# thevasudevgupta/gsoc-wav2vec2

Measured on AMD Instinct MI355X. Metric: audio-seconds/s (wav2vec2-base forward, 246000-sample pad), higher is better.
Workload: dtype f32

## Files before the change

gsoc-wav2vec2_amd/csrc/common.h:

```cpp
#pragma once

#include <hip/hip_runtime.h>
#include <stdint.h>
#include <stdio.h>

#include <atomic>
#include <initializer_list>
#include <type_traits>

#include <string>

#include "../../include/w2v2.h"

namespace w2v2 {

void set_error(const char* fmt, ...);

#define W2V2_HIP_CHECK(expr)                                                            \
    do {                                                                                \
        hipError_t _e = (expr);                                                         \
        if (_e != hipSuccess) {                                                         \
            ::w2v2::set_error("%s failed: %s (%s:%d)", #expr, hipGetErrorString(_e),    \
                              __FILE__, __LINE__);                                      \
            return W2V2_EHIP;                                                           \
// ... 95 lines not shown
    int outer_family;
    ProfScope(Profiler* p_, int family, double flops, double bytes, hipStream_t s_)
        : p(p_), tok((p_ && tl_prof_depth == 0) ? profiler_begin(p_, family, flops, bytes, s_) : -1), s(s_), outer_family(tl_launch_family) {
        if (tl_prof_depth++ == 0) tl_launch_family = family;
    }
    ~ProfScope() {
        if (--tl_prof_depth == 0) tl_launch_family = outer_family;
        if (tok >= 0) profiler_end(p, tok, s);
    }
};

extern thread_local Profiler* tl_step_prof;
struct StepProfScope {
    Profiler* outer;
    explicit StepProfScope(Profiler* p) : outer(tl_step_prof) { tl_step_prof = p; }
    ~StepProfScope() { tl_step_prof = outer; }
};

int launch_gemm(Profiler* prof, const float* A, int64_t lda, int64_t strideA, const float* B,
                int64_t ldb, float* C, int64_t ldc, int64_t strideC, const float* bias,
                const float* residual, int M, int N, int K, int nbatch, int act, hipStream_t s);

void gemm_f32_force_ring(int route);
bool gemm_f32_ring_ok(int tile, const float* A, int64_t lda, int64_t strideA, const float* B, int64_t ldb, int64_t strideB,
                      int M, int N, int K);
int launch_gemm_f32_ring(int tile, bool persist, const float* A, int64_t lda, int64_t strideA, const float* B, int64_t ldb,
                         int64_t strideB, float* C, int64_t ldc, int64_t strideC, const float* bias, const float* residual, int M,
                         int N, int K, int nbatch, int act, hipStream_t s);
int launch_gemm_f32_ring_split(bool persist, int64_t main_tiles, const float* A, int64_t lda, const float* B, int64_t ldb, float* C,
                               int64_t ldc, const float* bias, const float* residual, int M, int N, int K, int act, hipStream_t s);

int launch_gemm_bf16(Profiler* prof, const float* A, int64_t lda, int64_t strideA, const float* B, int64_t ldb,
                     int64_t strideB, float* C, int64_t ldc, int64_t strideC, const float* bias,
                     const float* residual, int M, int N, int K, int nbatch, int act, hipStream_t s);
bool gemm_split_supported(const float* A, int64_t lda, int64_t strideA, int M, int N, int K);
int launch_split_weight(const float* w, uint16_t* planes, int K, int N, hipStream_t s);
int launch_gemm_split(Profiler* prof, const float* A, int64_t lda, int64_t strideA, const uint16_t* planes, float* C, int64_t ldc,
                      int64_t strideC, const float* bias, const float* residual, int M, int N, int K, int nbatch, int act,
                      hipStream_t s);

bool gemm_split_sw_ok(const uint16_t* A16, int64_t planeA, int64_t lda, int64_t strideA, int M, int N, int K);
int launch_split_weight_sw(const float* w, uint16_t* img, int K, int N, int fmt, void* scratch, hipStream_t s);
int launch_split_planes(const float* x, uint16_t* planes, int64_t plane, int64_t n, int fmt, int* range_flag, hipStream_t s);
int launch_gemm_split_sw(Profiler* prof, int fmt, const uint16_t* A16, int64_t planeA, int64_t lda, int64_t strideA, const uint16_t* Bimg,
                         const float* out_scale, float* C, uint16_t* C16, int64_t planeC, int64_t ldc, int64_t strideC, const float* bias,
                         const float* residual, int M, int N, int K, int nbatch, int act, int* range_flag, hipStream_t s);

int launch_check_select_forms(unsigned long long* mismatches_dev , hipStream_t s);

struct GemmShadows {
    const uint16_t* A16 = nullptr;
    const uint16_t* B16 = nullptr;
    uint16_t* C16 = nullptr;
    int64_t ldb16 = 0;
    bool transA = false;
    int zmod = 0;
    int64_t strideB16 = 0, strideC2 = 0, strideBias = 0;
    int64_t strideB2 = 0;
    bool overlapA = false;
    int kseg = 0;
    int64_t segA = 0, segB = 0;
    float* colsum = nullptr;
    int64_t strideCS = 0;
    const uint16_t* B16p = nullptr;
    int64_t validK = 0;
    int kextra = 0;
    bool b_zero_row = false;
    int force_kernel = 0;
};
bool gemm_bf16_sw_ok(int M, int N, int K, int64_t lda, int64_t ldb16, int64_t strideA);
int launch_gemm_bf16_sw(const uint16_t* A16, int64_t lda, int64_t strideA, const uint16_t* B16, int64_t ldb16, float* C, uint16_t* C16,
// ... 207 lines not shown
    q = __builtin_fmaf(ax, q, 0x1.4515fap-1f);
    q = __builtin_fmaf(ax, q, 0x1.078e5p-3f);
    q = __builtin_fmaf(ax, q, ax);
    const float large = 1.0f - expf(-q);
    return copysignf(ax < 1.0f ? small : large, x);
}
__device__ __forceinline__ float tanh_select(float x) {
    const float ax = fabsf(x), t = x * x;
    float p = __builtin_fmaf(t, -0x1.758e7ap-8f, 0x1.521192p-6f);
    p = __builtin_fmaf(t, p, -0x1.b8389cp-5f);
    p = __builtin_fmaf(t, p, 0x1.110704p-3f);
    p = __builtin_fmaf(t, p, -0x1.555532p-2f);
    const float small = __builtin_fmaf(t, ax * p, ax);
    const float large = __builtin_fmaf(-2.0f, __builtin_amdgcn_rcpf(expf(ax * 2.0f) + 1.0f), 1.0f);
    return copysignf(ax < 0.625f ? small : large, x);
}
__device__ __forceinline__ float gelu_tanh_select(float x) {
    const float c = 0.79788456080286535588f;
    return 0.5f * x * (1.0f + tanh_select(c * (x + 0.044715f * x * x * x)));
}
__device__ __forceinline__ float gelu_erf_select(float x) {
    return 0.5f * x * (1.0f + erf_select(x * 0.70710678118654752440f));
}
__device__ __forceinline__ float gelu_tanh(float x) {
    const float c = 0.79788456080286535588f;
    return 0.5f * x * (1.0f + tanhf(c * (x + 0.044715f * x * x * x)));
}
__device__ __forceinline__ float gelu_erf_fast(float x) {
    const float z = fabsf(x) * 0.70710678118654752440f;
    const float t = __builtin_amdgcn_rcpf(fmaf(0.3275911f, z, 1.0f));
    float p = fmaf(1.061405429f, t, -1.453152027f);
    p = fmaf(p, t, 1.421413741f);
    p = fmaf(p, t, -0.284496736f);
    p = fmaf(p, t, 0.254829592f);
    const float e = __builtin_amdgcn_exp2f(-z * z * 1.44269504088896340736f);
    const float erf_abs = fmaf(-p * t, e, 1.0f);
    return 0.5f * x + 0.5f * fabsf(x) * erf_abs;
}

using f32x2_t = __attribute__((ext_vector_type(2))) float;
__device__ __forceinline__ f32x2_t gelu_erf_fast2(f32x2_t x) {
    const f32x2_t ax = {fabsf(x[0]), fabsf(x[1])};
    const f32x2_t z = ax * f32x2_t{0.70710678118654752440f, 0.70710678118654752440f};
    const f32x2_t d = __builtin_elementwise_fma(f32x2_t{0.3275911f, 0.3275911f}, z, f32x2_t{1.0f, 1.0f});
    const f32x2_t t = {__builtin_amdgcn_rcpf(d[0]), __builtin_amdgcn_rcpf(d[1])};
    f32x2_t q = __builtin_elementwise_fma(f32x2_t{1.061405429f, 1.061405429f}, t, f32x2_t{-1.453152027f, -1.453152027f});
// ... 105 lines not shown
```

gsoc-wav2vec2_amd/csrc/gemm_epilogue.h:

```cpp
#pragma once

#include "common.h"
#include "train.h"

namespace w2v2 {

#ifdef __HIPCC__
using f32x16_t = __attribute__((ext_vector_type(16))) float;

template <int MT, int NTL, bool FAST_GELU>
__device__ __forceinline__ void gemm_epilogue(const f32x16_t (&acc)[MT][NTL], float* __restrict__ C, uint16_t* __restrict__ C16,
                                              const float* __restrict__ R, const float* __restrict__ bias, int ldc,
                                              int rows_left, int cols_left, int act, int li, int lh, int64_t c16_plane = 0, int c16_fmt = 0,
                                              int* range_flag = nullptr) {
    bool ovf = false;
    const bool interior = rows_left >= MT * 32 && cols_left >= NTL * 32;
#pragma unroll
    for (int nt = 0; nt < NTL; ++nt) {
        const int cl = nt * 32 + li;
        const bool col_ok = cl < cols_left;
        const float bv = (bias && col_ok) ? bias[cl] : 0.0f;
#pragma unroll
        for (int mt = 0; mt < MT; ++mt) {
            f32x16_t v = acc[mt][nt];
#pragma unroll
            for (int r = 0; r < 16; ++r) v[r] += bv;
            if (act == 1) {
#pragma unroll
                for (int r = 0; r < 16; r += 2) {
                    if (FAST_GELU) {
                        const f32x2_t g = gelu_erf_fast2(f32x2_t{v[r], v[r + 1]});
                        v[r] = g[0];
                        v[r + 1] = g[1];
                    } else {
                        v[r] = gelu_erf(v[r]);
                        v[r + 1] = gelu_erf(v[r + 1]);
                    }
                }
            } else if (act == 2) {
#pragma unroll
                for (int r = 0; r < 16; ++r) v[r] = gelu_tanh(v[r]);
            }
            const int off0 = (mt * 32 + 4 * lh) * ldc + cl;
            if (interior) {
                if (R) {
#pragma unroll
                    for (int r = 0; r < 16; ++r) v[r] += R[off0 + ((r & 3) + 8 * (r >> 2)) * ldc];
                }
                if (C) {
#pragma unroll
                    for (int r = 0; r < 16; ++r) C[off0 + ((r & 3) + 8 * (r >> 2)) * ldc] = v[r];
                }
                if (C16) {
#pragma unroll
                    for (int r = 0; r < 16; ++r) {
                        uint16_t* const d = C16 + off0 + ((r & 3) + 8 * (r >> 2)) * ldc;
                        if (c16_plane && c16_fmt == PF_F16X2) split2h_one(v[r], F16X2_ACT_SCALE, d[0], d[c16_plane], ovf);
                        else if (c16_plane) split3_one(v[r], d[0], d[c16_plane], d[2 * c16_plane]);
                        else d[0] = (uint16_t)pack_bf16_rne(v[r], 0.0f);
                    }
                }
            } else if (col_ok) {
#pragma unroll
                for (int r = 0; r < 16; ++r) {
                    const int rl = mt * 32 + (r & 3) + 8 * (r >> 2) + 4 * lh;
                    if (rl < rows_left) {
                        const int off = off0 + ((r & 3) + 8 * (r >> 2)) * ldc;
                        float o = v[r];
                        if (R) o += R[off];
                        if (C) C[off] = o;
// ... 17 lines not shown
```

gsoc-wav2vec2_amd/csrc/gemm_f32.hip:

```cpp
#include <stdlib.h>


#include "common.h"
#include "gemm_epilogue.h"

namespace w2v2 {

using f32x16 = __attribute__((ext_vector_type(16))) float;
using f32x4 = __attribute__((ext_vector_type(4))) float;

namespace {

constexpr int BK = 32;
constexpr int LDA_S = BK + 4;

struct GemmArgs {
    const float* A;
    const float* B;
    float* C;
    const float* bias;
    const float* residual;
    int64_t lda, ldb, ldc, strideA, strideB, strideC;
    int M, N, K, act;
    int tiles_m, tiles_n;
// ... 324 lines not shown
    const int64_t n4 = (int64_t)M * N / 4;
    for (int64_t i = (int64_t)blockIdx.x * 256 + threadIdx.x; i < n4; i += (int64_t)gridDim.x * 256) {
        const int64_t e = i * 4, row = e / N;
        const int col = (int)(e % N);
        float4 acc = reinterpret_cast<const float4*>(slabs)[i];
        for (int z = 1; z < S; ++z) {
            const float4 v = reinterpret_cast<const float4*>(slabs + (int64_t)z * M * N)[i];
            acc.x += v.x; acc.y += v.y; acc.z += v.z; acc.w += v.w;
        }
        if (bias) { acc.x += bias[col]; acc.y += bias[col + 1]; acc.z += bias[col + 2]; acc.w += bias[col + 3]; }
        acc.x = apply_act(acc.x, act); acc.y = apply_act(acc.y, act); acc.z = apply_act(acc.z, act); acc.w = apply_act(acc.w, act);
        if (residual) {
            const float4 r = *reinterpret_cast<const float4*>(residual + row * ldc + col);
            acc.x += r.x; acc.y += r.y; acc.z += r.z; acc.w += r.w;
        }
        *reinterpret_cast<float4*>(C + row * ldc + col) = acc;
    }
}

thread_local int tl_precision = 0;
thread_local int tl_ring = -1;

constexpr int RING_DEFAULT = 2;
int ring_route() { return tl_ring >= 0 ? tl_ring : tune_int("W2V2_GEMM_RING", RING_DEFAULT); }

}

void gemm_set_precision(int mode) { tl_precision = mode; }
void gemm_f32_force_ring(int route) { tl_ring = route; }
int gemm_get_precision() { return tl_precision; }

int launch_gemm(Profiler* prof, const float* A, int64_t lda, int64_t strideA, const float* B,
                int64_t ldb, float* C, int64_t ldc, int64_t strideC, const float* bias,
                const float* residual, int M, int N, int K, int nbatch, int act, hipStream_t s) {
    return launch_gemm_ex(prof, A, lda, strideA, B, ldb, 0, C, ldc, strideC, bias, residual, M, N, K, nbatch, act, s);
}

int launch_gemm_ex(Profiler* prof, const float* A, int64_t lda, int64_t strideA, const float* B,
                   int64_t ldb, int64_t strideB, float* C, int64_t ldc, int64_t strideC, const float* bias,
                   const float* residual, int M, int N, int K, int nbatch, int act, hipStream_t s) {
    if (tl_precision == 1)
        return launch_gemm_bf16(prof, A, lda, strideA, B, ldb, strideB, C, ldc, strideC, bias, residual, M, N, K, nbatch, act, s);
    W2V2_REQUIRE(A && B && C, "gemm: null operand");
    W2V2_REQUIRE(M > 0 && N > 0 && K > 0 && nbatch > 0, "gemm: bad sizes M=%d N=%d K=%d batch=%d", M, N, K, nbatch);
    W2V2_REQUIRE(lda >= 1 && ldb >= N && ldc >= N && ldc < (1 << 23), "gemm: bad leading dimensions");
    W2V2_REQUIRE(act >= 0 && act <= 2, "gemm: bad activation %d", act);
    GemmArgs g;
    g.A = A; g.B = B; g.C = C; g.bias = bias; g.residual = residual;
    g.lda = lda; g.ldb = ldb; g.ldc = ldc; g.strideA = strideA; g.strideB = strideB; g.strideC = strideC;
    g.M = M; g.N = N; g.K = K; g.act = act;
    const bool fast = (K % BK == 0) && (N % 4 == 0) && (lda % 4 == 0) && (ldb % 4 == 0) &&
                      (strideA % 4 == 0) && (strideB % 4 == 0) && ((reinterpret_cast<uintptr_t>(A) & 15) == 0) &&
                      ((reinterpret_cast<uintptr_t>(B) & 15) == 0);
    ProfScope ps(prof, FAM_GEMM, 2.0 * M * (double)N * K * nbatch,
                 4.0 * nbatch * ((double)M * K + (double)M * N) + 4.0 * (double)K * N, s);
    int cfg = forced_cfg();
    const bool by_shape = cfg < 0;
    if (cfg < 0 && fast && nbatch == 1 && strideB == 0 && K >= 1024 && (ldc % 4) == 0 &&
        ((reinterpret_cast<uintptr_t>(C) | reinterpret_cast<uintptr_t>(residual) | reinterpret_cast<uintptr_t>(bias)) & 15) == 0) {
        const int64_t tiles64 = (int64_t)((M + 63) / 64) * ((N + 63) / 64);
        int S = 1;
        for (int cand = 8; cand >= 2; cand >>= 1)
            if (K % (cand * BK) == 0 && K / cand >= 256 && tiles64 * cand <= 512) { S = cand; break; }
        if (S > 1 && tiles64 <= 256) {
            const size_t need = (size_t)S * M * N;
            float* ws = nullptr;
            void* raw = nullptr;
            if (int e = stream_scratch(SCRATCH_SPLITK, s, need * sizeof(float), &raw)) return e;
            ws = reinterpret_cast<float*>(raw);
            GemmArgs h = g;
            h.C = ws; h.bias = nullptr; h.residual = nullptr; h.act = 0;
            h.K = K / S; h.strideA = K / S; h.strideB = (int64_t)(K / S) * ldb; h.ldc = N; h.strideC = (int64_t)M * N;
            if (int e = launch_dma<2, 2, 2, 32, 64, 64>(h, S, s)) return e;
            const int64_t n4 = (int64_t)M * N / 4;
            int64_t blocks = (n4 + 255) / 256;
            blocks = blocks > 2048 ? 2048 : blocks;
            W2V2_LAUNCH(splitk_reduce_kernel, dim3((unsigned)blocks), dim3(256), 0, s, ws, C, bias, residual, M, N, ldc, S, act);
            W2V2_HIP_CHECK(hipGetLastError());
// ... 87 lines not shown
```

gsoc-wav2vec2_amd/csrc/gemm_f32_sw.hip:

```cpp
#include "common.h"
#include "gemm_epilogue.h"
#include "gemm_sw_common.h"

namespace w2v2 {

namespace {

struct GemmRingArgs {
    const float* A;
    const float* B;
    float* C;
    const float* bias;
    const float* residual;
    int64_t lda, ldb, ldc, strideA, strideB, strideC;
    int M, N, K, act;
    int tiles_m, tiles_n, nbatch;
    int gm;
    int total;
    int first;
};

template <int WM, int WN, int BKT, int BM, int BN, int NS>
struct RingCfg {
    static constexpr int STAGE = (BM * BKT + BKT * BN) * 4;
    static constexpr int LDS = NS * STAGE;
    static constexpr int NW = WM * WN;
    static constexpr int NPA = BM * BKT / 256, NPB = BKT * BN / 256;
    static constexpr int PPA = NPA / NW, PPB = NPB / NW;
    static constexpr int P = PPA + PPB;
    static_assert(NPA % NW == 0 && NPB % NW == 0, "every wave issues the same number of pieces (counted waits)");
    static_assert((NS - 2) * P <= 63, "vmcnt field");
};

template <int WM, int WN, int BKT, int BM, int BN, int NS, bool QUAD = false>
__global__ __launch_bounds__(WM* WN * 64) __attribute__((amdgpu_waves_per_eu(4))) void gemm_f32_ring_kernel(GemmRingArgs g) {
    using R_ = RingCfg<WM, WN, BKT, BM, BN, NS>;
    constexpr int NW = R_::NW, PPA = R_::PPA, PPB = R_::PPB, P = R_::P, STAGE = R_::STAGE;
    constexpr int RPP = 256 / BKT;
    constexpr int SPR = BKT / 4;
    constexpr int SW = BKT == 32 ? 1 : 2;
    constexpr int WTM = BM / WM, WTN = BN / WN, MT = WTM / 32, NTL = WTN / 32;
    extern __shared__ __attribute__((aligned(16))) float smem[];
    const int tid = threadIdx.x, lane = tid & 63, wave = __builtin_amdgcn_readfirstlane(tid >> 6);
    const int wm = wave / WN, wn = wave % WN, li = lane & 31, lh = lane >> 5;
    const unsigned lds0 = (unsigned)(uintptr_t)(__attribute__((address_space(3))) float*)smem;

    const int nwg = g.tiles_m * g.tiles_n, total = g.total, G = gridDim.x;
    const int ntl = (total - (int)blockIdx.x + G - 1) / G;
    const int nk = g.K / BKT, nsteps = ntl * nk;
    auto tile_of = [&](int i, int& z, int& m0, int& n0) {
        const int v = (int)blockIdx.x + i * G;
        const int q = total >> 3, r = total & 7, xcd = v & 7, idx = v >> 3;
        int t = (xcd < r ? xcd * (q + 1) : r * (q + 1) + (xcd - r) * q) + idx;
        int sub = 0;
        if constexpr (QUAD) {
            sub = t & 3;
            t = g.first + (t >> 2);
// ... 89 lines not shown
#pragma unroll
                for (int mt = 0; mt < MT; ++mt)
#pragma unroll
                    for (int nt = 0; nt < NTL; ++nt)
                        acc[mt][nt] = __builtin_amdgcn_mfma_f32_32x32x2f32(a[mt][e], b[nt][e], acc[mt][nt], 0, 0, 0);
        }
    };
    auto ring_barrier = [&](bool counted) {
        if (counted) sw_wait_vm<(NS - 2) * P>();
        else sw_wait_vm<0>();
        __builtin_amdgcn_s_barrier();
        asm volatile("" ::: "memory");
        __builtin_amdgcn_sched_barrier(0);
    };

    set_issue_tile(0);
    for (int p = 0; p < NS - 1 && p < nsteps; ++p) issue_step();
    ring_barrier(nsteps >= NS - 1);
    __builtin_amdgcn_s_setprio(1);

    int s = 0, cst = 0;
    for (int ci = 0; ci < ntl; ++ci) {
        zero();
        for (int kt = 0; kt < nk; ++kt, ++s) {
            const bool more = s + NS - 1 < nsteps;
            if (more) issue_step();
            __builtin_amdgcn_sched_barrier(0);
            compute(cst);
            __builtin_amdgcn_sched_barrier(0);
            ring_barrier(more);
            cst = cst + 1 == NS ? 0 : cst + 1;
        }
        int z, m0, n0;
        tile_of(ci, z, m0, n0);
        const int64_t tile_off = (int64_t)z * g.strideC + (int64_t)(m0 + wm * WTM) * g.ldc + (n0 + wn * WTN);
        int act = g.act, ldc = (int)g.ldc, eli = li, elh = lh;
        const float* res = g.residual;
        const float* bias = g.bias;
        asm volatile("" : "+s"(act), "+s"(res), "+s"(bias), "+s"(ldc), "+v"(eli), "+v"(elh));
        __builtin_amdgcn_s_setprio(0);
        gemm_epilogue<MT, NTL, false>(acc, g.C + tile_off, nullptr, res ? res + tile_off : nullptr, bias ? bias + (n0 + wn * WTN) : nullptr,
                                     ldc, g.M - (m0 + wm * WTM), g.N - (n0 + wn * WTN), act, eli, elh);
        __builtin_amdgcn_s_setprio(1);
    }
    __builtin_amdgcn_s_setprio(0);
}

template <int WM, int WN, int BKT, int BM, int BN, int NS, bool QUAD = false>
int launch_ring(GemmRingArgs& g, bool persist, hipStream_t s, int64_t first = -1, int gm = 0) {
    using R_ = RingCfg<WM, WN, BKT, BM, BN, NS>;
    static_assert(2 * R_::LDS <= 160 * 1024, "two blocks per CU");
    constexpr int TM = QUAD ? 2 * BM : BM, TN = QUAD ? 2 * BN : BN;
    g.tiles_m = (g.M + TM - 1) / TM;
    g.tiles_n = (g.N + TN - 1) / TN;
    int64_t total = (int64_t)g.tiles_m * g.tiles_n * g.nbatch;
    W2V2_REQUIRE(first < 0 || (first > 0 && first < total && g.nbatch == 1 && g.M % TM == 0 && g.N % TN == 0), "gemm ring: bad split");
    W2V2_REQUIRE(!QUAD || first > 0, "gemm ring: quarter tiles need a split");
    g.first = QUAD ? (int)first : 0;
    if (first > 0) total = QUAD ? 4 * (total - first) : first;
    W2V2_REQUIRE(total < (1ll << 31), "gemm ring: %lld tiles", (long long)total);
    g.total = (int)total;
    constexpr int PER_CU = WM * WN == 8 ? 2 : 160 * 1024 / R_::LDS > 4 ? 4 : 160 * 1024 / R_::LDS;
    int grid = (int)total;
    if (persist) {
        int dev = 0, cus = 0;
        W2V2_HIP_CHECK(hipGetDevice(&dev));
        W2V2_HIP_CHECK(hipDeviceGetAttribute(&cus, hipDeviceAttributeMultiprocessorCount, dev));
        const int resident = (PER_CU * cus) & ~7;
        if (resident >= 8 && total > resident) grid = resident;
    }
    g.gm = first > 0 ? gm : g.nbatch == 1 ? tile_group_rows(g.tiles_m, g.tiles_n, (int64_t)BM * g.K * 4, BM == 256 ? 96 : 32 * PER_CU) : 0;
    static std::atomic<bool> attr_set{false};
    if (!attr_set) {
        W2V2_HIP_CHECK(hipFuncSetAttribute(reinterpret_cast<const void*>(gemm_f32_ring_kernel<WM, WN, BKT, BM, BN, NS, QUAD>),
                                           hipFuncAttributeMaxDynamicSharedMemorySize, R_::LDS));
        attr_set = true;
    }
    W2V2_LAUNCH((gemm_f32_ring_kernel<WM, WN, BKT, BM, BN, NS, QUAD>), dim3(grid), dim3(WM * WN * 64), R_::LDS, s, g);
    W2V2_HIP_CHECK(hipGetLastError());
    return W2V2_OK;
}

}

bool gemm_f32_ring_ok(int tile, const float* A, int64_t lda, int64_t strideA, const float* B, int64_t ldb, int64_t strideB,
                      int M, int N, int K) {
    const int BM = tile == 0 ? 256 : tile == 1 ? 128 : 64, BKT = tile == 2 ? 32 : 16;
    const bool align = ((reinterpret_cast<uintptr_t>(A) | reinterpret_cast<uintptr_t>(B)) & 15) == 0 && lda % 4 == 0 &&
                       ldb % 4 == 0 && strideA % 4 == 0 && strideB % 4 == 0;
    return align && K % BKT == 0 && N % 4 == 0 && N >= 4 && (int64_t)BM * lda * 4 < (1ll << 31) &&
           (int64_t)BKT * ldb * 4 < (1ll << 31) && M > 0;
}

int launch_gemm_f32_ring(int tile, bool persist, const float* A, int64_t lda, int64_t strideA, const float* B, int64_t ldb,
                         int64_t strideB, float* C, int64_t ldc, int64_t strideC, const float* bias, const float* residual, int M,
                         int N, int K, int nbatch, int act, hipStream_t s) {
    W2V2_REQUIRE(tile >= 0 && tile <= 2, "gemm ring: tile %d", tile);
    W2V2_REQUIRE(gemm_f32_ring_ok(tile, A, lda, strideA, B, ldb, strideB, M, N, K), "gemm ring: unsupported shape M=%d N=%d K=%d", M, N, K);
    GemmRingArgs g;
    g.A = A; g.B = B; g.C = C; g.bias = bias; g.residual = residual;
    g.lda = lda; g.ldb = ldb; g.ldc = ldc; g.strideA = strideA; g.strideB = strideB; g.strideC = strideC;
    g.M = M; g.N = N; g.K = K; g.act = act; g.nbatch = nbatch;
    if (tile == 0) return launch_ring<4, 2, 16, 256, 128, 3>(g, persist, s);
    if (tile == 1) return launch_ring<2, 4, 16, 128, 128, 4>(g, persist, s);
    return launch_ring<2, 2, 32, 64, 64, 3>(g, persist, s);
}

int launch_gemm_f32_ring_split(bool persist, int64_t main_tiles, const float* A, int64_t lda, const float* B, int64_t ldb, float* C,
                               int64_t ldc, const float* bias, const float* residual, int M, int N, int K, int act, hipStream_t s) {
    W2V2_REQUIRE(M % 128 == 0 && N % 128 == 0 && gemm_f32_ring_ok(1, A, lda, 0, B, ldb, 0, M, N, K) && gemm_f32_ring_ok(2, A, lda, 0, B, ldb, 0, M, N, K),
                 "gemm ring split: unsupported shape M=%d N=%d K=%d", M, N, K);
    GemmRingArgs g;
    g.A = A; g.B = B; g.C = C; g.bias = bias; g.residual = residual;
    g.lda = lda; g.ldb = ldb; g.ldc = ldc; g.strideA = 0; g.strideB = 0; g.strideC = 0;
    g.M = M; g.N = N; g.K = K; g.act = act; g.nbatch = 1;
    const int gm = tile_group_rows(M / 128, N / 128, (int64_t)128 * K * 4, 64);
    if (int e = launch_ring<2, 4, 16, 128, 128, 4>(g, persist, s, main_tiles, gm)) return e;
    return launch_ring<2, 2, 32, 64, 64, 3, true>(g, false, s, main_tiles, gm);
}

}
```

gsoc-wav2vec2_amd/csrc/selftest.hip:

```cpp
#include "common.h"

namespace w2v2 {

namespace {

__global__ __launch_bounds__(256) void select_forms_kernel(unsigned long long* mismatches ) {
    unsigned long long bad_erf = 0, bad_tanh = 0;
    const uint64_t stride = (uint64_t)gridDim.x * 256;
    for (uint64_t i = (uint64_t)blockIdx.x * 256 + threadIdx.x; i < (1ull << 32); i += stride) {
        const float x = __uint_as_float((unsigned)i);
        const float a = erff(x), b = erf_select(x);
        if (__float_as_uint(a) != __float_as_uint(b) && !(a != a && b != b)) ++bad_erf;
        const float c = tanhf(x), d = tanh_select(x);
        if (__float_as_uint(c) != __float_as_uint(d) && !(c != c && d != d)) ++bad_tanh;
    }
    if (bad_erf) atomicAdd(&mismatches[0], bad_erf);
    if (bad_tanh) atomicAdd(&mismatches[1], bad_tanh);
}

}

int launch_check_select_forms(unsigned long long* mismatches_dev, hipStream_t s) {
    W2V2_REQUIRE(mismatches_dev, "check_select_forms: null argument");
    W2V2_HIP_CHECK(hipMemsetAsync(mismatches_dev, 0, 2 * sizeof(unsigned long long), s));
    W2V2_LAUNCH(select_forms_kernel, dim3(4096), dim3(256), 0, s, mismatches_dev);
    W2V2_HIP_CHECK(hipGetLastError());
    return W2V2_OK;
}

}
```

gsoc-wav2vec2_amd/csrc/w2v2_api.hip:

```cpp
#include <algorithm>
#include <mutex>
#include <atomic>
#include <stdarg.h>
#include <stdlib.h>
#include <string.h>

#include <map>
#include <string>
#include <unordered_map>
#include <vector>

#include "common.h"
#include "model.h"

namespace w2v2 {

static thread_local char g_err[1024] = "";
void set_error(const char* fmt, ...) {
    va_list ap;
    va_start(ap, fmt);
    vsnprintf(g_err, sizeof(g_err), fmt, ap);
    va_end(ap);
}

// ... 693 lines not shown
    W2V2_REQUIRE(variant != 2 || gemm_bf16_sw_ok(M, N, K, lda, K, strideA),
                 "op_gemm_bf16_shadows: variant 2 needs N %% 256 == 0, K %% 64 == 0, K >= 192 and 16-byte aligned rows");
    GemmShadows x;
    x.A16 = A16; x.B16 = B16; x.C16 = C16; x.ldb16 = K; x.force_kernel = variant;
    return launch_gemm_bf16_x(nullptr, nullptr, lda, strideA, nullptr, N, 0, C, ldc, strideC, bias, residual, M, N, K, nbatch, act, x,
                              reinterpret_cast<hipStream_t>(stream));
}
int w2v2_op_gemm_split(const float* A, int64_t lda, int64_t strideA, const float* B, float* C, int64_t ldc, int64_t strideC,
                       const float* bias, const float* residual, int32_t M, int32_t N, int32_t K, int32_t nbatch, int32_t act,
                       void* stream) {
    W2V2_REQUIRE(A && B && C && N > 0 && K > 0, "op_gemm_split: null operand");
    hipStream_t s = reinterpret_cast<hipStream_t>(stream);
    uint16_t* planes = nullptr;
    W2V2_HIP_CHECK(hipMalloc(reinterpret_cast<void**>(&planes), (size_t)3 * K * N * sizeof(uint16_t)));
    int e = launch_split_weight(B, planes, K, N, s);
    if (!e) e = launch_gemm_split(nullptr, A, lda, strideA, planes, C, ldc, strideC, bias, residual, M, N, K, nbatch, act, s);
    (void)hipStreamSynchronize(s);
    (void)hipFree(planes);
    return e;
}
int w2v2_op_check_select_forms(uint64_t* mismatches, void* stream) {
    return launch_check_select_forms(reinterpret_cast<unsigned long long*>(mismatches), reinterpret_cast<hipStream_t>(stream));
}
int w2v2_op_split_planes(const float* x, uint16_t* planes, int64_t plane_stride, int64_t n, int32_t fmt, int32_t* range_flag, void* stream) {
    W2V2_REQUIRE(fmt == PF_BF16X3 || fmt == PF_F16X2, "op_split_planes: unknown plane format %d", fmt);
    return launch_split_planes(x, planes, plane_stride, n, fmt, range_flag, reinterpret_cast<hipStream_t>(stream));
}
int w2v2_op_split_weight(const float* B, uint16_t* images, float* scale_ws, int32_t K, int32_t N, int32_t fmt, void* stream) {
    W2V2_REQUIRE(fmt == PF_BF16X3 || fmt == PF_F16X2, "op_split_weight: unknown plane format %d", fmt);
    return launch_split_weight_sw(B, images, K, N, fmt, scale_ws, reinterpret_cast<hipStream_t>(stream));
}
int w2v2_op_gemm_split_planes(int32_t fmt, const uint16_t* A16, int64_t planeA, int64_t lda, int64_t strideA, const uint16_t* Bimg,
                              const float* out_scale, float* C, uint16_t* C16, int64_t planeC, int64_t ldc, int64_t strideC,
                              const float* bias, const float* residual, int32_t M, int32_t N, int32_t K, int32_t nbatch, int32_t act,
                              int32_t* range_flag, void* stream) {
    return launch_gemm_split_sw(nullptr, fmt, A16, planeA, lda, strideA, Bimg, out_scale, C, C16, planeC, ldc, strideC, bias, residual, M, N, K,
                                nbatch, act, range_flag, reinterpret_cast<hipStream_t>(stream));
}
int w2v2_op_gemm_bf16_at(const float* At, int64_t lda, int64_t strideA, const float* B, int64_t ldb, int64_t strideB,
                         float* C, int64_t ldc, int64_t strideC, int32_t M, int32_t N, int32_t K, int32_t nbatch, void* stream) {
    GemmShadows x;
    x.transA = true;
    return launch_gemm_bf16_x(nullptr, At, lda, strideA, B, ldb, strideB, C, ldc, strideC, nullptr, nullptr, M, N, K, nbatch, 0, x,
                              reinterpret_cast<hipStream_t>(stream));
}
uint32_t w2v2_crc32c_extend(uint32_t crc, const void* data, uint64_t n) {
// ... 125 lines not shown
```

gsoc-wav2vec2_amd/wav2vec2/_native.py:

```python

import ctypes as C
import os

_HERE = os.path.dirname(os.path.abspath(__file__))
_PKG_ROOT = os.path.dirname(_HERE)
LIB_PATH = os.path.join(_PKG_ROOT, "lib", "libw2v2.so")

MAX_CONV_LAYERS = 16
ALIGN_MAX_LABELS = 8191
SCORE_MAX_LABELS = 8191
SPOT_MAX_LABELS = 256
BEAM_MAX_WIDTH = 64
BEAM_MAX_VOCAB = 64
CUTS_CHUNK = 1024
CUTS_MAX_FRAMES = 1 << 24
RESAMPLE_TILE = 2048
RESAMPLE_MAX_L = 4096
RESAMPLE_MAX_TABLE = 1 << 22
EDIT_MAX_LEN = 65535
WORDLM_MAX_ORDER = 5
BIAS_MAX_STATES = 1 << 20


class W2V2Config(C.Structure):
# ... 113 lines not shown
    "w2v2_pos_conv_dw_bf16_ws_floats": (C.c_int, [_I32, _I32, _I32, _I32, _I32, C.POINTER(_I64), C.POINTER(_I32)]),
    "w2v2_op_pos_conv_dw_bf16": (C.c_int, [_P, _P, _P, _P, _P, _P, _P, _I32, _I32, _I32, _I32, _I32, _P]),
    "w2v2_op_weight_norm_bwd": (C.c_int, [_P, _P, _P, _P, _P, _I32, _I32, _I32, _I32, _P]),
    "w2v2_activation_info": (C.c_int, [_P, C.c_char_p, C.POINTER(_I64)]),
    "w2v2_copy_activation": (C.c_int, [_P, C.c_char_p, _P, _I64, _P]),
    "w2v2_profile_enable": (C.c_int, [_P, C.c_int]),
    "w2v2_profile_families": (C.c_int, [_P, C.c_uint32]),
    "w2v2_profile_sampling": (C.c_int, [_P, C.c_int32]),
    "w2v2_profile_seen": (C.c_int, [_P, C.c_int, C.POINTER(_I64)]),
    "w2v2_profile_kernel_launches": (C.c_int, [_P, C.c_int, C.POINTER(_I64)]),
    "w2v2_profile_num_families": (C.c_int, []),
    "w2v2_clock_probe": (C.c_int, [_P, _I32, _P, C.POINTER(_I32)]),
    "w2v2_profile_read": (C.c_int, [_P, C.c_int, C.POINTER(C.c_char_p), C.POINTER(_I64),
                                    C.POINTER(C.c_double), C.POINTER(C.c_double), C.POINTER(C.c_double)]),
    "w2v2_profile_reset": (C.c_int, [_P]),
    "w2v2_op_gemm": (C.c_int, [_P, _I64, _I64, _P, _I64, _P, _I64, _I64, _P, _P, _I32, _I32, _I32, _I32, _I32, _P]),
    "w2v2_op_gemm_variant": (C.c_int, [_P, _I64, _I64, _P, _I64, _P, _I64, _I64, _P, _P, _I32, _I32, _I32, _I32, _I32, _I32, _P]),
    "w2v2_op_set_precision": (C.c_int, [_I32]),
    "w2v2_op_gemm_split": (C.c_int, [_P, _I64, _I64, _P, _P, _I64, _I64, _P, _P, _I32, _I32, _I32, _I32, _I32, _P]),
    "w2v2_op_gemm_bf16_at": (C.c_int, [_P, _I64, _I64, _P, _I64, _I64, _P, _I64, _I64, _I32, _I32, _I32, _I32, _P]),
    "w2v2_crc32c_extend": (C.c_uint32, [C.c_uint32, _P, C.c_uint64]),
    "w2v2_op_weight_grad_bf16": (C.c_int, [_P, _P, _P, _I64, _I32, _I32, _I32, _I32, _I32, _P]),
    "w2v2_op_check_select_forms": (C.c_int, [_P, _P]),
    "w2v2_op_split_planes": (C.c_int, [_P, _P, _I64, _I64, _I32, _P, _P]),
    "w2v2_op_split_weight": (C.c_int, [_P, _P, _P, _I32, _I32, _I32, _P]),
    "w2v2_op_gemm_split_planes": (C.c_int, [_I32, _P, _I64, _I64, _I64, _P, _P, _P, _P, _I64, _I64, _I64, _P, _P, _I32, _I32, _I32, _I32, _I32, _P, _P]),
    "w2v2_op_gemm_bf16_shadows": (C.c_int, [_P, _I64, _I64, _P, _P, _P, _I64, _I64, _P, _P, _I32, _I32, _I32, _I32, _I32, _I32, _P]),
    "w2v2_op_gemm_bf16": (C.c_int, [_P, _I64, _I64, _P, _I64, _P, _I64, _I64, _P, _P, _I32, _I32, _I32, _I32, _I32, _P]),
    "w2v2_op_layer_norm": (C.c_int, [_P, _P, _P, _P, _I64, _I32, C.c_float, _I32, _P]),
    "w2v2_conv0_ws_floats": (_I64, [_I32, _I64, _I32, _I32, _I32]),
    "w2v2_op_conv0": (C.c_int, [_P, _P, _P, _P, _P, _P, _P, _I32, _I64, _I32, _I32, _I32, C.c_float, _I32, _I32, _P]),
    "w2v2_op_weight_norm_regroup": (C.c_int, [_P, _P, _P, _I32, _I32, _I32, _I32, _P]),
    "w2v2_op_pos_conv": (C.c_int, [_P, _P, _P, _P, _P, _I32, _I32, _I32, _I32, _I32, _I32, _P]),
    "w2v2_op_attention": (C.c_int, [_P, _P, _P, _I32, _I32, _I32, _I32, _P]),
    "w2v2_op_attention_packed": (C.c_int, [_P, _I32, _P, _P, _P, _I64, _P, _I32, _I32, _P]),
    "w2v2_op_frame_lengths": (C.c_int, [_P, _P, _I32, _I64, C.POINTER(_I32), C.POINTER(_I32), _I32, _P]),
    "w2v2_op_normalize_windows": (C.c_int, [_P, _I32, _P, _P, _P, _P]),
}

_lib = None


class NativeLibraryError(RuntimeError):
    pass


# ... 84 lines not shown
```

include/w2v2.h:

```cpp
#ifndef W2V2_H_
#define W2V2_H_

#include <stdint.h>

#ifdef __cplusplus
extern "C" {
#endif

#define W2V2_MAX_CONV_LAYERS 16

enum {
    W2V2_OK = 0,
    W2V2_EINVAL = -1,
    W2V2_ENOTFOUND = -2,
    W2V2_EHIP = -3,
    W2V2_ESTATE = -4
};

typedef struct w2v2_config {
    int32_t vocab_size;
    int32_t hidden_size;
    int32_t num_heads;
    int32_t num_layers;
    int32_t intermediate_size;
// ... 234 lines not shown

int w2v2_op_gemm_bf16_shadows(const uint16_t* A16_dev, int64_t lda, int64_t strideA, const uint16_t* B16_nk_dev, float* C_dev,
                              uint16_t* C16_dev, int64_t ldc, int64_t strideC, const float* bias_dev, const float* residual_dev,
                              int32_t M, int32_t N, int32_t K, int32_t nbatch, int32_t act, int32_t variant, void* stream);

int w2v2_op_gemm_split(const float* A_dev, int64_t lda, int64_t strideA, const float* B_dev,
                       float* C_dev, int64_t ldc, int64_t strideC,
                       const float* bias_dev, const float* residual_dev,
                       int32_t M, int32_t N, int32_t K, int32_t nbatch, int32_t act, void* stream);

#define W2V2_PLANES_BF16X3 0
#define W2V2_PLANES_F16X2 1
int w2v2_op_split_planes(const float* x_dev, uint16_t* planes_dev, int64_t plane_stride, int64_t n, int32_t fmt, int32_t* range_flag_dev,
                         void* stream);
int w2v2_op_split_weight(const float* B_dev, uint16_t* images_dev, float* scale_ws_dev, int32_t K, int32_t N, int32_t fmt, void* stream);
int w2v2_op_gemm_split_planes(int32_t fmt, const uint16_t* A16_dev, int64_t planeA, int64_t lda, int64_t strideA,
                              const uint16_t* B_images_dev, const float* out_scale_dev,
                              float* C_dev, uint16_t* C16_dev, int64_t planeC, int64_t ldc, int64_t strideC,
                              const float* bias_dev, const float* residual_dev,
                              int32_t M, int32_t N, int32_t K, int32_t nbatch, int32_t act, int32_t* range_flag_dev, void* stream);

int w2v2_op_check_select_forms(uint64_t* mismatches_dev, void* stream);

int w2v2_op_gemm_bf16_at(const float* At_dev, int64_t lda, int64_t strideA,
                         const float* B_dev, int64_t ldb, int64_t strideB,
                         float* C_dev, int64_t ldc, int64_t strideC,
                         int32_t M, int32_t N, int32_t K, int32_t nbatch, void* stream);

int w2v2_op_weight_grad_bf16(const uint16_t* x16_dev, const uint16_t* dy16_dev, float* slabs_dev,
                             int64_t rows, int32_t Kin, int32_t Nout, int32_t rows_per_slab, int32_t nslabs, int32_t variant,
                             void* stream);

uint32_t w2v2_crc32c_extend(uint32_t crc, const void* data_host, uint64_t n);

int w2v2_op_layer_norm(const float* x_dev, float* y_dev, const float* gamma_dev,
                       const float* beta_dev, int64_t rows, int32_t C, float eps,
                       int32_t act, void* stream);

int64_t w2v2_conv0_ws_floats(int32_t B, int64_t L, int32_t K, int32_t stride, int32_t C);
int w2v2_op_conv0(const float* wave_dev, const float* kernel_dev, const float* bias_dev,
                  const float* gamma_dev, const float* beta_dev, float* out_dev,
                  float* stats_ws_dev, int32_t B, int64_t L, int32_t K, int32_t stride,
                  int32_t C, float eps, int32_t norm_mode, int32_t act, void* stream);

int w2v2_op_weight_norm_regroup(const float* weight_v_dev, const float* weight_g_dev,
                                float* wg_dev, int32_t K, int32_t cg, int32_t H,
// ... 70 lines not shown
```

Before: 8292.

## Specialize ring GEMM kernel per epilogue form and inline exact-bit GELU

```diff
diff --git a/gsoc-wav2vec2_amd/csrc/common.h b/gsoc-wav2vec2_amd/csrc/common.h
--- a/gsoc-wav2vec2_amd/csrc/common.h
+++ b/gsoc-wav2vec2_amd/csrc/common.h
@@ -141,6 +141,8 @@
                 const float* residual, int M, int N, int K, int nbatch, int act, hipStream_t s);
 
 void gemm_f32_force_ring(int route);
+bool gemm_f32_ring_form_ok(const float* bias, const float* residual, int act);
+void gemm_f32_ring_launches(int64_t* counts );
 bool gemm_f32_ring_ok(int tile, const float* A, int64_t lda, int64_t strideA, const float* B, int64_t ldb, int64_t strideB,
                       int M, int N, int K);
 int launch_gemm_f32_ring(int tile, bool persist, const float* A, int64_t lda, int64_t strideA, const float* B, int64_t ldb,
@@ -166,6 +168,8 @@
                          const float* residual, int M, int N, int K, int nbatch, int act, int* range_flag, hipStream_t s);
 
 int launch_check_select_forms(unsigned long long* mismatches_dev , hipStream_t s);
+int launch_check_gelu_epilogue(unsigned long long* mismatches_dev , hipStream_t s);
+int launch_gelu_reference(const float* x, float* y, int64_t n, hipStream_t s);
 
 struct GemmShadows {
     const uint16_t* A16 = nullptr;
@@ -419,6 +423,28 @@
 __device__ __forceinline__ float gelu_erf_select(float x) {
     return 0.5f * x * (1.0f + erf_select(x * 0.70710678118654752440f));
 }
+__device__ __forceinline__ float gelu_erf_epi(float x) {
+    const float z = x * 0.70710678118654752440f, az = fabsf(z), t = z * z;
+    float p = __builtin_fmaf(t, -0x1.268bc2p-11f, 0x1.420828p-8f);
+    p = __builtin_fmaf(t, p, -0x1.b5937p-6f);
+    p = __builtin_fmaf(t, p, 0x1.ce077cp-4f);
+    p = __builtin_fmaf(t, p, -0x1.81266p-2f);
+    p = __builtin_fmaf(t, p, 0x1.06ebap-3f);
+    const float small = __builtin_fmaf(az, p, az);
+    const float ac = __builtin_fminf(az, 4.0f);
+    float q = __builtin_fmaf(ac, 0x1.1d3156p-16f, -0x1.8d129p-12f);
+    q = __builtin_fmaf(ac, q, 0x1.f9a6d2p-9f);
+    q = __builtin_fmaf(ac, q, -0x1.8c3164p-6f);
+    q = __builtin_fmaf(ac, q, 0x1.b4e9c8p-4f);
+    q = __builtin_fmaf(ac, q, 0x1.4515fap-1f);
+    q = __builtin_fmaf(ac, q, 0x1.078e5p-3f);
+    q = __builtin_fmaf(ac, q, ac);
+    const float ph = q * -0x1.715476p+0f;
+    const float pl = __builtin_fmaf(q, -0x1.4ae0bep-26f, __builtin_fmaf(q, -0x1.715476p+0f, -ph));
+    const float e = __builtin_rintf(ph);
+    const float large = 1.0f - __builtin_amdgcn_ldexpf(__builtin_amdgcn_exp2f((ph - e) + pl), (int)e);
+    return 0.5f * x * (1.0f + copysignf(az < 1.0f ? small : large, z));
+}
 __device__ __forceinline__ float gelu_tanh(float x) {
     const float c = 0.79788456080286535588f;
     return 0.5f * x * (1.0f + tanhf(c * (x + 0.044715f * x * x * x)));
diff --git a/gsoc-wav2vec2_amd/csrc/gemm_epilogue.h b/gsoc-wav2vec2_amd/csrc/gemm_epilogue.h
--- a/gsoc-wav2vec2_amd/csrc/gemm_epilogue.h
+++ b/gsoc-wav2vec2_amd/csrc/gemm_epilogue.h
@@ -8,13 +8,22 @@
 #ifdef __HIPCC__
 using f32x16_t = __attribute__((ext_vector_type(16))) float;
 
-template <int MT, int NTL, bool FAST_GELU>
+template <int MT, int NTL, bool FAST_GELU, bool RES_AHEAD = false>
 __device__ __forceinline__ void gemm_epilogue(const f32x16_t (&acc)[MT][NTL], float* __restrict__ C, uint16_t* __restrict__ C16,
                                               const float* __restrict__ R, const float* __restrict__ bias, int ldc,
                                               int rows_left, int cols_left, int act, int li, int lh, int64_t c16_plane = 0, int c16_fmt = 0,
                                               int* range_flag = nullptr) {
     bool ovf = false;
     const bool interior = rows_left >= MT * 32 && cols_left >= NTL * 32;
+    f32x16_t rv[RES_AHEAD ? MT * NTL : 1];
+    if (RES_AHEAD && interior) {
+#pragma unroll
+        for (int nt = 0; nt < NTL; ++nt)
+#pragma unroll
+            for (int mt = 0; mt < MT; ++mt)
+#pragma unroll
+                for (int r = 0; r < 16; ++r) rv[nt * MT + mt][r] = R[(mt * 32 + 4 * lh + (r & 3) + 8 * (r >> 2)) * ldc + nt * 32 + li];
+    }
 #pragma unroll
     for (int nt = 0; nt < NTL; ++nt) {
         const int cl = nt * 32 + li;
@@ -26,16 +35,16 @@
 #pragma unroll
             for (int r = 0; r < 16; ++r) v[r] += bv;
             if (act == 1) {
+                if (FAST_GELU) {
 #pragma unroll
-                for (int r = 0; r < 16; r += 2) {
-                    if (FAST_GELU) {
+                    for (int r = 0; r < 16; r += 2) {
                         const f32x2_t g = gelu_erf_fast2(f32x2_t{v[r], v[r + 1]});
                         v[r] = g[0];
                         v[r + 1] = g[1];
-                    } else {
-                        v[r] = gelu_erf(v[r]);
-                        v[r + 1] = gelu_erf(v[r + 1]);
                     }
+                } else {
+#pragma unroll
+                    for (int r = 0; r < 16; ++r) v[r] = gelu_erf_epi(v[r]);
                 }
             } else if (act == 2) {
 #pragma unroll
@@ -45,7 +54,7 @@
             if (interior) {
                 if (R) {
 #pragma unroll
-                    for (int r = 0; r < 16; ++r) v[r] += R[off0 + ((r & 3) + 8 * (r >> 2)) * ldc];
+                    for (int r = 0; r < 16; ++r) v[r] += RES_AHEAD ? rv[RES_AHEAD ? nt * MT + mt : 0][r] : R[off0 + ((r & 3) + 8 * (r >> 2)) * ldc];
                 }
                 if (C) {
 #pragma unroll
diff --git a/gsoc-wav2vec2_amd/csrc/gemm_f32.hip b/gsoc-wav2vec2_amd/csrc/gemm_f32.hip
--- a/gsoc-wav2vec2_amd/csrc/gemm_f32.hip
+++ b/gsoc-wav2vec2_amd/csrc/gemm_f32.hip
@@ -370,7 +370,7 @@
 thread_local int tl_ring = -1;
 
 constexpr int RING_DEFAULT = 2;
-int ring_route() { return tl_ring >= 0 ? tl_ring : tune_int("W2V2_GEMM_RING", RING_DEFAULT); }
+int ring_route_any() { return tl_ring >= 0 ? tl_ring : tune_int("W2V2_GEMM_RING", RING_DEFAULT); }
 
 }
 
@@ -402,6 +402,7 @@
                       ((reinterpret_cast<uintptr_t>(B) & 15) == 0);
     ProfScope ps(prof, FAM_GEMM, 2.0 * M * (double)N * K * nbatch,
                  4.0 * nbatch * ((double)M * K + (double)M * N) + 4.0 * (double)K * N, s);
+    auto ring_route = [&]() { return gemm_f32_ring_form_ok(bias, residual, act) ? ring_route_any() : 0; };
     int cfg = forced_cfg();
     const bool by_shape = cfg < 0;
     if (cfg < 0 && fast && nbatch == 1 && strideB == 0 && K >= 1024 && (ldc % 4) == 0 &&
diff --git a/gsoc-wav2vec2_amd/csrc/gemm_f32_sw.hip b/gsoc-wav2vec2_amd/csrc/gemm_f32_sw.hip
--- a/gsoc-wav2vec2_amd/csrc/gemm_f32_sw.hip
+++ b/gsoc-wav2vec2_amd/csrc/gemm_f32_sw.hip
@@ -13,7 +13,7 @@
     const float* bias;
     const float* residual;
     int64_t lda, ldb, ldc, strideA, strideB, strideC;
-    int M, N, K, act;
+    int M, N, K;
     int tiles_m, tiles_n, nbatch;
     int gm;
     int total;
@@ -32,7 +32,7 @@
     static_assert((NS - 2) * P <= 63, "vmcnt field");
 };
 
-template <int WM, int WN, int BKT, int BM, int BN, int NS, bool QUAD = false>
+template <int WM, int WN, int BKT, int BM, int BN, int NS, bool QUAD, bool BIAS, bool GELU, bool RES>
 __global__ __launch_bounds__(WM* WN * 64) __attribute__((amdgpu_waves_per_eu(4))) void gemm_f32_ring_kernel(GemmRingArgs g) {
     using R_ = RingCfg<WM, WN, BKT, BM, BN, NS>;
     constexpr int NW = R_::NW, PPA = R_::PPA, PPB = R_::PPB, P = R_::P, STAGE = R_::STAGE;
@@ -168,6 +168,8 @@
     int s = 0, cst = 0;
     for (int ci = 0; ci < ntl; ++ci) {
         zero();
+        int z, m0, n0;
+        tile_of(ci, z, m0, n0);
         for (int kt = 0; kt < nk; ++kt, ++s) {
             const bool more = s + NS - 1 < nsteps;
             if (more) issue_step();
@@ -177,23 +179,21 @@
             ring_barrier(more);
             cst = cst + 1 == NS ? 0 : cst + 1;
         }
-        int z, m0, n0;
-        tile_of(ci, z, m0, n0);
         const int64_t tile_off = (int64_t)z * g.strideC + (int64_t)(m0 + wm * WTM) * g.ldc + (n0 + wn * WTN);
-        int act = g.act, ldc = (int)g.ldc, eli = li, elh = lh;
-        const float* res = g.residual;
-        const float* bias = g.bias;
-        asm volatile("" : "+s"(act), "+s"(res), "+s"(bias), "+s"(ldc), "+v"(eli), "+v"(elh));
+        int ldc = (int)g.ldc, eli = li, elh = lh;
+        asm volatile("" : "+s"(ldc), "+v"(eli), "+v"(elh));
         __builtin_amdgcn_s_setprio(0);
-        gemm_epilogue<MT, NTL, false>(acc, g.C + tile_off, nullptr, res ? res + tile_off : nullptr, bias ? bias + (n0 + wn * WTN) : nullptr,
-                                     ldc, g.M - (m0 + wm * WTM), g.N - (n0 + wn * WTN), act, eli, elh);
+        gemm_epilogue<MT, NTL, false, RES && MT * NTL <= 2>(acc, g.C + tile_off, nullptr, RES ? g.residual + tile_off : nullptr, BIAS ? g.bias + (n0 + wn * WTN) : nullptr,
+                                     ldc, g.M - (m0 + wm * WTM), g.N - (n0 + wn * WTN), GELU ? 1 : 0, eli, elh);
         __builtin_amdgcn_s_setprio(1);
     }
     __builtin_amdgcn_s_setprio(0);
 }
 
-template <int WM, int WN, int BKT, int BM, int BN, int NS, bool QUAD = false>
-int launch_ring(GemmRingArgs& g, bool persist, hipStream_t s, int64_t first = -1, int gm = 0) {
+std::atomic<int64_t> g_ring_launches[4];
+
+template <int WM, int WN, int BKT, int BM, int BN, int NS, bool QUAD, bool BIAS, bool GELU, bool RES>
+int launch_ring_form(GemmRingArgs& g, bool persist, hipStream_t s, int64_t first, int gm) {
     using R_ = RingCfg<WM, WN, BKT, BM, BN, NS>;
     static_assert(2 * R_::LDS <= 160 * 1024, "two blocks per CU");
     constexpr int TM = QUAD ? 2 * BM : BM, TN = QUAD ? 2 * BN : BN;
@@ -218,15 +218,41 @@
     g.gm = first > 0 ? gm : g.nbatch == 1 ? tile_group_rows(g.tiles_m, g.tiles_n, (int64_t)BM * g.K * 4, BM == 256 ? 96 : 32 * PER_CU) : 0;
     static std::atomic<bool> attr_set{false};
     if (!attr_set) {
-        W2V2_HIP_CHECK(hipFuncSetAttribute(reinterpret_cast<const void*>(gemm_f32_ring_kernel<WM, WN, BKT, BM, BN, NS, QUAD>),
+        W2V2_HIP_CHECK(hipFuncSetAttribute(reinterpret_cast<const void*>(gemm_f32_ring_kernel<WM, WN, BKT, BM, BN, NS, QUAD, BIAS, GELU, RES>),
                                            hipFuncAttributeMaxDynamicSharedMemorySize, R_::LDS));
         attr_set = true;
     }
-    W2V2_LAUNCH((gemm_f32_ring_kernel<WM, WN, BKT, BM, BN, NS, QUAD>), dim3(grid), dim3(WM * WN * 64), R_::LDS, s, g);
+    W2V2_LAUNCH((gemm_f32_ring_kernel<WM, WN, BKT, BM, BN, NS, QUAD, BIAS, GELU, RES>), dim3(grid), dim3(WM * WN * 64), R_::LDS, s, g);
     W2V2_HIP_CHECK(hipGetLastError());
+    g_ring_launches[QUAD ? 3 : BM == 256 ? 0 : BM == 128 ? 1 : 2].fetch_add(1, std::memory_order_relaxed);
     return W2V2_OK;
 }
 
+int ring_form(const float* bias, const float* residual, int act) {
+    if (act == 1) return residual ? -1 : bias ? 2 : 5;
+    if (act != 0) return -1;
+    return residual ? (bias ? 3 : 4) : (bias ? 1 : 0);
+}
+
+template <int WM, int WN, int BKT, int BM, int BN, int NS, bool QUAD = false>
+int launch_ring(GemmRingArgs& g, int act, bool persist, hipStream_t s, int64_t first = -1, int gm = 0) {
+    switch (ring_form(g.bias, g.residual, act)) {
+        case 0: return launch_ring_form<WM, WN, BKT, BM, BN, NS, QUAD, false, false, false>(g, persist, s, first, gm);
+        case 1: return launch_ring_form<WM, WN, BKT, BM, BN, NS, QUAD, true, false, false>(g, persist, s, first, gm);
+        case 2: return launch_ring_form<WM, WN, BKT, BM, BN, NS, QUAD, true, true, false>(g, persist, s, first, gm);
+        case 3: return launch_ring_form<WM, WN, BKT, BM, BN, NS, QUAD, true, false, true>(g, persist, s, first, gm);
+        case 4: return launch_ring_form<WM, WN, BKT, BM, BN, NS, QUAD, false, false, true>(g, persist, s, first, gm);
+        case 5: return launch_ring_form<WM, WN, BKT, BM, BN, NS, QUAD, false, true, false>(g, persist, s, first, gm);
+    }
+    W2V2_REQUIRE(false, "gemm ring: no instance for this epilogue (bias %d, residual %d, act %d)", g.bias != nullptr, g.residual != nullptr, act);
+    return W2V2_OK;
+}
+
+}
+
+bool gemm_f32_ring_form_ok(const float* bias, const float* residual, int act) { return ring_form(bias, residual, act) >= 0; }
+void gemm_f32_ring_launches(int64_t* counts) {
+    for (int i = 0; i < 4; ++i) counts[i] = g_ring_launches[i].load(std::memory_order_relaxed);
 }
 
 bool gemm_f32_ring_ok(int tile, const float* A, int64_t lda, int64_t strideA, const float* B, int64_t ldb, int64_t strideB,
@@ -246,10 +272,10 @@
     GemmRingArgs g;
     g.A = A; g.B = B; g.C = C; g.bias = bias; g.residual = residual;
     g.lda = lda; g.ldb = ldb; g.ldc = ldc; g.strideA = strideA; g.strideB = strideB; g.strideC = strideC;
-    g.M = M; g.N = N; g.K = K; g.act = act; g.nbatch = nbatch;
-    if (tile == 0) return launch_ring<4, 2, 16, 256, 128, 3>(g, persist, s);
-    if (tile == 1) return launch_ring<2, 4, 16, 128, 128, 4>(g, persist, s);
-    return launch_ring<2, 2, 32, 64, 64, 3>(g, persist, s);
+    g.M = M; g.N = N; g.K = K; g.nbatch = nbatch;
+    if (tile == 0) return launch_ring<4, 2, 16, 256, 128, 3>(g, act, persist, s);
+    if (tile == 1) return launch_ring<2, 4, 16, 128, 128, 4>(g, act, persist, s);
+    return launch_ring<2, 2, 32, 64, 64, 3>(g, act, persist, s);
 }
 
 int launch_gemm_f32_ring_split(bool persist, int64_t main_tiles, const float* A, int64_t lda, const float* B, int64_t ldb, float* C,
@@ -259,10 +285,10 @@
     GemmRingArgs g;
     g.A = A; g.B = B; g.C = C; g.bias = bias; g.residual = residual;
     g.lda = lda; g.ldb = ldb; g.ldc = ldc; g.strideA = 0; g.strideB = 0; g.strideC = 0;
-    g.M = M; g.N = N; g.K = K; g.act = act; g.nbatch = 1;
+    g.M = M; g.N = N; g.K = K; g.nbatch = 1;
     const int gm = tile_group_rows(M / 128, N / 128, (int64_t)128 * K * 4, 64);
-    if (int e = launch_ring<2, 4, 16, 128, 128, 4>(g, persist, s, main_tiles, gm)) return e;
-    return launch_ring<2, 2, 32, 64, 64, 3, true>(g, false, s, main_tiles, gm);
-}
-
-}
+    if (int e = launch_ring<2, 4, 16, 128, 128, 4>(g, act, persist, s, main_tiles, gm)) return e;
+    return launch_ring<2, 2, 32, 64, 64, 3, true>(g, act, false, s, main_tiles, gm);
+}
+
+}
diff --git a/gsoc-wav2vec2_amd/csrc/selftest.hip b/gsoc-wav2vec2_amd/csrc/selftest.hip
--- a/gsoc-wav2vec2_amd/csrc/selftest.hip
+++ b/gsoc-wav2vec2_amd/csrc/selftest.hip
@@ -18,6 +18,23 @@
     if (bad_tanh) atomicAdd(&mismatches[1], bad_tanh);
 }
 
+__global__ __launch_bounds__(256) void gelu_epilogue_kernel(unsigned long long* mismatches ) {
+    unsigned long long bad_epi = 0, bad_sel = 0;
+    const uint64_t stride = (uint64_t)gridDim.x * 256;
+    for (uint64_t i = (uint64_t)blockIdx.x * 256 + threadIdx.x; i < (1ull << 32); i += stride) {
+        const float x = __uint_as_float((unsigned)i);
+        const float a = gelu_erf(x), b = gelu_erf_epi(x), c = gelu_erf_select(x);
+        if (__float_as_uint(a) != __float_as_uint(b) && !(a != a && b != b)) ++bad_epi;
+        if (__float_as_uint(a) != __float_as_uint(c) && !(a != a && c != c)) ++bad_sel;
+    }
+    if (bad_epi) atomicAdd(&mismatches[0], bad_epi);
+    if (bad_sel) atomicAdd(&mismatches[1], bad_sel);
+}
+
+__global__ __launch_bounds__(256) void gelu_reference_kernel(const float* __restrict__ x, float* __restrict__ y, int64_t n) {
+    for (int64_t i = (int64_t)blockIdx.x * 256 + threadIdx.x; i < n; i += (int64_t)gridDim.x * 256) y[i] = gelu_erf(x[i]);
+}
+
 }
 
 int launch_check_select_forms(unsigned long long* mismatches_dev, hipStream_t s) {
@@ -28,4 +45,20 @@
     return W2V2_OK;
 }
 
+int launch_check_gelu_epilogue(unsigned long long* mismatches_dev, hipStream_t s) {
+    W2V2_REQUIRE(mismatches_dev, "check_gelu_epilogue: null argument");
+    W2V2_HIP_CHECK(hipMemsetAsync(mismatches_dev, 0, 2 * sizeof(unsigned long long), s));
+    W2V2_LAUNCH(gelu_epilogue_kernel, dim3(4096), dim3(256), 0, s, mismatches_dev);
+    W2V2_HIP_CHECK(hipGetLastError());
+    return W2V2_OK;
 }
+
+int launch_gelu_reference(const float* x, float* y, int64_t n, hipStream_t s) {
+    W2V2_REQUIRE(x && y && n > 0, "gelu_reference: bad argument");
+    const int64_t blocks = (n + 255) / 256;
+    W2V2_LAUNCH(gelu_reference_kernel, dim3((unsigned)(blocks > 4096 ? 4096 : blocks)), dim3(256), 0, s, x, y, n);
+    W2V2_HIP_CHECK(hipGetLastError());
+    return W2V2_OK;
+}
+
+}
diff --git a/gsoc-wav2vec2_amd/csrc/w2v2_api.hip b/gsoc-wav2vec2_amd/csrc/w2v2_api.hip
--- a/gsoc-wav2vec2_amd/csrc/w2v2_api.hip
+++ b/gsoc-wav2vec2_amd/csrc/w2v2_api.hip
@@ -739,6 +739,17 @@
 int w2v2_op_check_select_forms(uint64_t* mismatches, void* stream) {
     return launch_check_select_forms(reinterpret_cast<unsigned long long*>(mismatches), reinterpret_cast<hipStream_t>(stream));
 }
+int w2v2_op_check_gelu_epilogue(uint64_t* mismatches, void* stream) {
+    return launch_check_gelu_epilogue(reinterpret_cast<unsigned long long*>(mismatches), reinterpret_cast<hipStream_t>(stream));
+}
+int w2v2_op_gelu_reference(const float* x, float* y, int64_t n, void* stream) {
+    return launch_gelu_reference(x, y, n, reinterpret_cast<hipStream_t>(stream));
+}
+int w2v2_op_gemm_ring_launches(int64_t* counts) {
+    W2V2_REQUIRE(counts, "op_gemm_ring_launches: null argument");
+    gemm_f32_ring_launches(counts);
+    return W2V2_OK;
+}
 int w2v2_op_split_planes(const float* x, uint16_t* planes, int64_t plane_stride, int64_t n, int32_t fmt, int32_t* range_flag, void* stream) {
     W2V2_REQUIRE(fmt == PF_BF16X3 || fmt == PF_F16X2, "op_split_planes: unknown plane format %d", fmt);
     return launch_split_planes(x, planes, plane_stride, n, fmt, range_flag, reinterpret_cast<hipStream_t>(stream));
diff --git a/gsoc-wav2vec2_amd/wav2vec2/_native.py b/gsoc-wav2vec2_amd/wav2vec2/_native.py
--- a/gsoc-wav2vec2_amd/wav2vec2/_native.py
+++ b/gsoc-wav2vec2_amd/wav2vec2/_native.py
@@ -159,6 +159,9 @@
     "w2v2_crc32c_extend": (C.c_uint32, [C.c_uint32, _P, C.c_uint64]),
     "w2v2_op_weight_grad_bf16": (C.c_int, [_P, _P, _P, _I64, _I32, _I32, _I32, _I32, _I32, _P]),
     "w2v2_op_check_select_forms": (C.c_int, [_P, _P]),
+    "w2v2_op_check_gelu_epilogue": (C.c_int, [_P, _P]),
+    "w2v2_op_gelu_reference": (C.c_int, [_P, _P, _I64, _P]),
+    "w2v2_op_gemm_ring_launches": (C.c_int, [C.POINTER(_I64)]),
     "w2v2_op_split_planes": (C.c_int, [_P, _P, _I64, _I64, _I32, _P, _P]),
     "w2v2_op_split_weight": (C.c_int, [_P, _P, _P, _I32, _I32, _I32, _P]),
     "w2v2_op_gemm_split_planes": (C.c_int, [_I32, _P, _I64, _I64, _I64, _P, _P, _P, _P, _I64, _I64, _I64, _P, _P, _I32, _I32, _I32, _I32, _I32, _P, _P]),
diff --git a/include/w2v2.h b/include/w2v2.h
--- a/include/w2v2.h
+++ b/include/w2v2.h
@@ -280,6 +280,10 @@
 
 int w2v2_op_check_select_forms(uint64_t* mismatches_dev, void* stream);
 
+int w2v2_op_check_gelu_epilogue(uint64_t* mismatches_dev, void* stream);
+int w2v2_op_gelu_reference(const float* x_dev, float* y_dev, int64_t n, void* stream);
+int w2v2_op_gemm_ring_launches(int64_t* counts);
+
 int w2v2_op_gemm_bf16_at(const float* At_dev, int64_t lda, int64_t strideA,
                          const float* B_dev, int64_t ldb, int64_t strideB,
                          float* C_dev, int64_t ldc, int64_t strideC,
```

After: 8410, median of 6. 1.01x the previous value.
